# ArmingLou/seed-vc

Hardware: AMD Instinct MI355X
Metric: mel_frames_per_sec (higher is better)
Workload: dtype f16; 1 GPU; seed-uvit-tat-xlsr-tiny CFM 25 steps cfg 0.7 + HiFT, batch 64 x (P=430,S=430) per GPU; batch_per_gpu=64, global_batch=64, prompt_frames=430, diffusion_steps=25, vocoder_precision=fp16p8, lanes_per_gpu=2, parallelism=utterance-sharded x1, audio gather on rank 0

## Files before the change

### include/seedvc_hip.h

```cpp
#ifndef SEEDVC_HIP_H
#define SEEDVC_HIP_H

#include <stdint.h>

#ifdef __cplusplus
extern "C" {
#endif

#define SVC_ABI_VERSION 1

typedef struct svc_tensor_desc {
    const char* name;
    const float* data;
    int ndim;
    int64_t shape[4];
} svc_tensor_desc_t;

typedef struct svc_dit_config {
    int version;
    int hidden_dim, num_heads, depth, in_channels, content_dim, style_dim;
    int final_layer_type;
    int time_as_token, style_as_token, uvit_skip_connection, long_skip_connection, style_condition;
    int wn_hidden_dim, wn_num_layers, wn_kernel_size, wn_dilation_rate;
} svc_dit_config_t;
// ... 65 lines not shown
    int in_channels, base_channels, nb_harmonics, sampling_rate;
    float nsf_alpha, nsf_sigma, nsf_voiced_threshold;
    int num_upsamples, upsample_rates[4], upsample_kernel_sizes[4];
    int istft_n_fft, istft_hop;
    int num_kernels, resblock_kernel_sizes[4], resblock_dilation_sizes[4][3];
    int source_resblock_kernel_sizes[4], source_resblock_dilation_sizes[4][3];
    float lrelu_slope, audio_limit;
    int f0_cond_channels;
    int precision;
} svc_hift_config_t;
typedef struct svc_hift svc_hift_t;
int svc_hift_create(const svc_hift_config_t* cfg, const svc_tensor_desc_t* weights, int n_weights,
                    void* stream, svc_hift_t** out);
void svc_hift_destroy(svc_hift_t* m);
int svc_hift_forward(svc_hift_t* m, const float* mel, const float* f0, const float* phase0, const float* noise,
                     int B, int S, float* out, float* f0_out, void* stream);
int svc_hift_forward_ragged(svc_hift_t* m, const float* mel, const int32_t* lens, const float* f0, const float* phase0,
                            const float* noise, int B, int S, float* out, float* f0_out, void* stream);
int svc_hift_forward_seeded(svc_hift_t* m, const float* mel, const int32_t* lens, const float* f0, const uint64_t* seeds, int B,
                            int S, float* out, float* f0_out, void* stream);
int svc_hift_noise_draws(uint64_t seed, int NH, long n, float* phase0, float* noise, void* stream);
int svc_bigvgan_set_microbatch(svc_bigvgan_t* m, int utterances);
int svc_hift_set_microbatch(svc_hift_t* m, int utterances);

typedef struct svc_ar_config {
    int dim, n_head, n_local_heads, head_dim, n_layer, intermediate_size, vocab_size, max_seq_len;
    float rope_base, norm_eps;
} svc_ar_config_t;
typedef struct svc_ar svc_ar_t;
int svc_ar_create(const svc_ar_config_t* cfg, const svc_tensor_desc_t* weights, int n_weights, void* stream, svc_ar_t** out);
void svc_ar_destroy(svc_ar_t* m);
int svc_ar_reset(svc_ar_t* m, void* stream);
int svc_ar_forward_generate(svc_ar_t* m, const float* x, int S, const int64_t* input_pos, const int64_t* kv_pos,
                            float* logits_out, void* stream);
int svc_ar_decode_step(svc_ar_t* m, const float* x, int set_pos, int64_t input_pos, int64_t kv_pos, float* logits_out,
                       void* stream);
int svc_ar_generate(svc_ar_t* m, const float* x_prefill, int S, const int64_t* input_pos, const int64_t* kv_pos,
                    const float* exp_noise, int max_new, int min_tokens_before_eos, float temperature, float top_p,
                    float repetition_penalty, int check_every, int32_t* tokens_out, int32_t* n_tokens, void* stream);
int svc_ar_set_max_batch(svc_ar_t* m, int max_batch, void* stream);
int svc_ar_prefill_slot(svc_ar_t* m, int slot, const float* x, int S, const int64_t* input_pos, const int64_t* kv_pos,
                        float* logits_out, void* stream);
int svc_ar_decode_step_batch(svc_ar_t* m, int B, const float* x, int set_pos, const int64_t* input_pos, const int64_t* kv_pos,
                             float* logits_out, void* stream);
int svc_ar_generate_batch(svc_ar_t* m, int B, const float* x_prefill, const int32_t* S, const int64_t* input_pos,
                          const int64_t* kv_pos, const float* exp_noise, int max_new, int min_tokens_before_eos, float temperature,
// ... 428 lines not shown
```

### seed-vc_amd/_lib.py

```python
import ctypes as C
import os

import torch

_HERE = os.path.dirname(os.path.abspath(__file__))
LIB_PATH = os.path.join(_HERE, "libseedvc_hip.so")

EXPORTS = [
    "svc_abi_version", "svc_last_error",
    "svc_dit_create", "svc_dit_destroy", "svc_dit_set_microbatch", "svc_dit_set_fused_min_rows", "svc_dit_set_fused_seams", "svc_dit_fused_available", "svc_dit_set_graphs", "svc_cfm_sample", "svc_dit_forward",
    "svc_cfm_sample_seeded", "svc_cfm_noise_draws", "svc_cfm_sample_rows", "svc_cfm_rows_plan", "svc_hift_forward_seeded", "svc_hift_noise_draws",
    "svc_bigvgan_create", "svc_bigvgan_destroy", "svc_bigvgan_forward", "svc_bigvgan_forward_ragged", "svc_bigvgan_set_microbatch",
    "svc_hift_create", "svc_hift_destroy", "svc_hift_forward", "svc_hift_forward_ragged", "svc_hift_set_microbatch",
    "svc_anti_alias_act_fwd",
    "svc_ar_create", "svc_ar_destroy", "svc_ar_reset", "svc_ar_forward_generate", "svc_ar_decode_step", "svc_ar_sample", "svc_ar_generate",
    "svc_ar_set_max_batch", "svc_ar_prefill_slot", "svc_ar_decode_step_batch", "svc_ar_generate_batch",
    "svc_ar_generate_batch_seeded", "svc_ar_exp_draws", "svc_v2_assemble_cond", "svc_mel_strip_prompt",
    "svc_ar_prefill_batch", "svc_ar_set_prefill_rows", "svc_ar_prefill_passes", "svc_ar_admit", "svc_ar_run", "svc_ar_retire",
    "svc_ar_session_active",
    "svc_lr_create", "svc_lr_destroy", "svc_lr_forward", "svc_crossfade",
    "svc_chunks_gather_cond", "svc_chunks_assemble", "svc_sola_step", "svc_rt_push", "svc_rt_push_tiles", "svc_rt_ring_floats",
    "svc_rt_out", "svc_rt_push_gated", "svc_rt_out_dev", "svc_rt_pitch_state_words", "svc_rt_pitch",
    "svc_rt_pitch_cache_words", "svc_rt_pitch_ring_words", "svc_rt_pitch_win",
    "svc_vad_create", "svc_vad_destroy", "svc_vad_rows", "svc_vad_history", "svc_vad_state_floats", "svc_vad_scores", "svc_vad_detect",
    "svc_vad_step",
    "svc_campplus_create", "svc_campplus_destroy", "svc_campplus_forward", "svc_kaldi_fbank_frames", "svc_kaldi_fbank",
    "svc_kaldi_fbank_ragged", "svc_campplus_forward_ragged",
    "svc_mel_create", "svc_mel_destroy", "svc_mel_frames", "svc_mel_forward", "svc_mel_forward_ragged", "svc_mel_min_len",
    "svc_resampler_create", "svc_resampler_destroy", "svc_resample_len", "svc_resampler_tile", "svc_resample",
    "svc_rmvpe_create", "svc_rmvpe_destroy", "svc_rmvpe_frames", "svc_rmvpe_min_len", "svc_rmvpe_set_plane_budget", "svc_rmvpe_set_timing", "svc_rmvpe_last_timing", "svc_rmvpe_mel",
    "svc_rmvpe_salience", "svc_rmvpe_decode", "svc_rmvpe_f0", "svc_f0_adjust",
    "svc_whisper_create", "svc_whisper_destroy", "svc_whisper_n_windows", "svc_whisper_rows", "svc_whisper_set_window_group",
    "svc_whisper_set_timing", "svc_whisper_last_timing", "svc_whisper_mel", "svc_whisper_encode", "svc_whisper_content",
    "svc_w2v_create", "svc_w2v_destroy", "svc_w2v_frames", "svc_w2v_n_windows", "svc_w2v_rows", "svc_w2v_set_window_group",
    "svc_w2v_set_timing", "svc_w2v_last_timing", "svc_w2v_normalize", "svc_w2v_features", "svc_w2v_posconv", "svc_w2v_encode",
    "svc_w2v_content", "svc_w2v_create_ex",
# ... 389 lines not shown
```

### seed-vc_amd/csrc/attention.hip

```cpp
#include <stdlib.h>

#include <type_traits>

#include "common.h"

namespace svc {
namespace {

constexpr int KT = 64;
constexpr int ROWB = 128;

__device__ __forceinline__ int lds_off(int row, int c16) { return row * ROWB + ((c16 ^ ((row >> 1) & 7)) << 4); }

__device__ __forceinline__ half_t out16(float acc, float inv) {
    float r = acc * inv;
    asm volatile("" : "+v"(r));
    return (half_t)r;
}

template <int QT, bool VPERM, bool OUT32 = false>
__global__ __launch_bounds__(256) void attn_kernel(const AttnParams p) {
    constexpr int BQ = 64 * QT;
    constexpr int NS = 3;
    __shared__ __attribute__((aligned(16))) char smem[NS * 2 * KT * ROWB];
    const int tid = threadIdx.x, lane = tid & 63, wave = tid >> 6;
    const int fr = lane & 15, fq = lane >> 4;
    const int nblk = gridDim.x, bid = blockIdx.x;
    const int xq = nblk >> 3, xr = nblk & 7, xcd = bid & 7;
    const int lid = (xcd < xr ? xcd * (xq + 1) : xr * (xq + 1) + (xcd - xr) * xq) + (bid >> 3);
    const int nqt = (p.Tq - p.q_start + BQ - 1) / BQ;
    const int qt_idx = lid % nqt;
    const int sh_idx = lid / nqt;
    const int h = sh_idx % p.H, seq = sh_idx / p.H;
    const int q0 = p.q_start + qt_idx * BQ + wave * 16 * QT;
    const long row_base = (long)seq * p.seq_rows;
    const int kv_len = p.kv_len ? p.kv_len[seq] : p.kv_len_const;
    const int n_kt = (kv_len + KT - 1) / KT;

    half8 qf[QT][2];
#pragma unroll
    for (int qt = 0; qt < QT; ++qt) {
        int qr = q0 + qt * 16 + fr;
        qr = qr < p.seq_rows ? qr : p.seq_rows - 1;
        const half_t* src = p.q + (row_base + qr) * p.ld_qk + h * 64 + fq * 8;
// ... 23 lines not shown
    const half_t* kcol[2];
    const half_t* vp[2];
#pragma unroll
    for (int j = 0; j < 2; ++j) {
        srow[j] = (wave * 2 + j) * 8 + (lane >> 3);
        const int cs = (lane & 7) ^ ((srow[j] >> 1) & 7);
        kcol[j] = p.k + row_base * p.ld_qk + h * 64 + cs * 8;
        vp[j] = p.vt + (long)seq * p.vt_seq_stride + (long)(h * 64 + srow[j]) * p.vt_ld + cs * 8;
    }
    auto issue_tile = [&](int kt) {
        char* kb = smem + (kt % NS) * 2 * KT * ROWB + wave_u * 2048;
#pragma unroll
        for (int j = 0; j < 2; ++j) {
            int kr = kt * KT + srow[j];
            kr = kr < p.seq_rows ? kr : p.seq_rows - 1;
            __builtin_amdgcn_global_load_lds((gptr_t)(kcol[j] + (long)kr * p.ld_qk), (lptr_t)(kb + j * 1024), 16, 0, 0);
            __builtin_amdgcn_global_load_lds((gptr_t)(vp[j] + kt * KT), (lptr_t)(kb + KT * ROWB + j * 1024), 16, 0, 0);
        }
    };
#pragma unroll
    for (int s_ = 0; s_ < NS - 1; ++s_)
        if (s_ < n_kt) issue_tile(s_);

    auto tile = [&](const int kt, auto mask_tag) {
        constexpr bool MASK = decltype(mask_tag)::value;
        wait_tiles<NS - 2, 4>(n_kt - 1 - kt);
        asm volatile("s_barrier" ::: "memory");
        if (kt + NS - 1 < n_kt) issue_tile(kt + NS - 1);
        const char* kb = smem + (kt % NS) * 2 * KT * ROWB;
        const char* vb = kb + KT * ROWB;

        float4v acc_s[4][QT];
#pragma unroll
        for (int i = 0; i < 4; ++i)
#pragma unroll
            for (int j = 0; j < QT; ++j) acc_s[i][j] = (float4v){-m_run[j], -m_run[j], -m_run[j], -m_run[j]};
#pragma unroll
        for (int ks = 0; ks < 2; ++ks) {
#pragma unroll
            for (int mt = 0; mt < 4; ++mt) {
                const half8 kf = *reinterpret_cast<const half8*>(kb + lds_off(mt * 16 + fr, ks * 4 + fq));
#pragma unroll
                for (int qt = 0; qt < QT; ++qt)
                    acc_s[mt][qt] = __builtin_amdgcn_mfma_f32_16x16x32_f16(kf, qf[qt][ks], acc_s[mt][qt], 0, 0, 0);
            }
        }
        if constexpr (MASK) {
#pragma unroll
            for (int mt = 0; mt < 4; ++mt)
#pragma unroll
                for (int r = 0; r < 4; ++r) {
                    const int key = kt * KT + mt * 16 + fq * 4 + r;
                    if (key >= kv_len) {
#pragma unroll
                        for (int qt = 0; qt < QT; ++qt) acc_s[mt][qt][r] = -1e30f;
                    }
                }
        }
#pragma unroll
        for (int qt = 0; qt < QT; ++qt) {
            float a = -1e30f;
#pragma unroll
            for (int mt = 0; mt < 4; ++mt)
                a = fmaxf(a, fmaxf(fmaxf(acc_s[mt][qt][0], acc_s[mt][qt][1]), fmaxf(acc_s[mt][qt][2], acc_s[mt][qt][3])));
            if (__builtin_expect(kt == 0 || __any(a > THR), 0)) {
                a = fmaxf(a, __shfl_xor(a, 16));
                a = fmaxf(a, __shfl_xor(a, 32));
                const float delta = kt == 0 ? a : (a > THR ? a : 0.f);
                const float alpha = __builtin_amdgcn_exp2f(-delta);
                m_run[qt] += delta;
                acc_l[qt] *= alpha;
#pragma unroll
                for (int dt = 0; dt < 4; ++dt) acc_o[dt][qt] *= alpha;
#pragma unroll
                for (int mt = 0; mt < 4; ++mt) acc_s[mt][qt] -= delta;
            }
        }
#pragma unroll
        for (int ks = 0; ks < 2; ++ks) {
            half8 pf[QT];
#pragma unroll
            for (int qt = 0; qt < QT; ++qt) {
                u32x4 u;
#pragma unroll
                for (int hh = 0; hh < 2; ++hh) {
                    const float4v sv = acc_s[2 * ks + hh][qt];
                    const float e0 = __builtin_amdgcn_exp2f(sv[0]), e1 = __builtin_amdgcn_exp2f(sv[1]);
                    const float e2 = __builtin_amdgcn_exp2f(sv[2]), e3 = __builtin_amdgcn_exp2f(sv[3]);
                    u[2 * hh] = __builtin_bit_cast(unsigned, __builtin_amdgcn_cvt_pkrtz(e0, e1));
                    u[2 * hh + 1] = __builtin_bit_cast(unsigned, __builtin_amdgcn_cvt_pkrtz(e2, e3));
                }
                pf[qt] = __builtin_bit_cast(half8, u);
                acc_l[qt] = __builtin_amdgcn_mfma_f32_16x16x32_f16(ones_f, pf[qt], acc_l[qt], 0, 0, 0);
            }
#pragma unroll
            for (int dt = 0; dt < 4; ++dt) {
                const int d = dt * 16 + fr;
                half8 vf;
                if constexpr (VPERM) {
                    vf = *reinterpret_cast<const half8*>(vb + lds_off(d, ks * 4 + fq));
                } else {
                    const int base = lds_off(d, ks * 4 + (fq >> 1)) + (fq & 1) * 8;
                    const int base2 = lds_off(d, ks * 4 + 2 + (fq >> 1)) + (fq & 1) * 8;
                    const half4 v0 = *reinterpret_cast<const half4*>(vb + base);
                    const half4 v1 = *reinterpret_cast<const half4*>(vb + base2);
#pragma unroll
                    for (int e = 0; e < 4; ++e) { vf[e] = v0[e]; vf[4 + e] = v1[e]; }
                }
#pragma unroll
                for (int qt = 0; qt < QT; ++qt)
                    acc_o[dt][qt] = __builtin_amdgcn_mfma_f32_16x16x32_f16(vf, pf[qt], acc_o[dt][qt], 0, 0, 0);
            }
        }
    };
    const bool ragged = (kv_len % KT) != 0;
    const int n_full = ragged ? n_kt - 1 : n_kt;
    for (int kt = 0; kt < n_full; ++kt) tile(kt, std::false_type{});
    if (ragged) tile(n_kt - 1, std::true_type{});
    asm volatile("s_waitcnt vmcnt(0)" ::: "memory");

#pragma unroll
    for (int qt = 0; qt < QT; ++qt) {
        const float l = __shfl(acc_l[qt][0], fr);
        const float inv = l > 0.f ? 1.0f / l : 0.f;
        const int qr = q0 + qt * 16 + fr;
        if constexpr (OUT32) {
          if (qr < p.Tq) {
            float* dst = p.out32 + (row_base + qr) * p.ld_out + h * 64 + fq * 4;
#pragma unroll
            for (int dt = 0; dt < 4; ++dt)
                *reinterpret_cast<float4v*>(dst + dt * 16) =
                    (float4v){acc_o[dt][qt][0] * inv, acc_o[dt][qt][1] * inv, acc_o[dt][qt][2] * inv, acc_o[dt][qt][3] * inv};
          }
        } else if (qr < p.Tq) {
            half_t* dst = p.out + (row_base + qr) * p.ld_out + h * 64 + fq * 4;
#pragma unroll
            for (int dt = 0; dt < 4; ++dt) {
                half4 o = {out16(acc_o[dt][qt][0], inv), out16(acc_o[dt][qt][1], inv),
                           out16(acc_o[dt][qt][2], inv), out16(acc_o[dt][qt][3], inv)};
                *reinterpret_cast<half4*>(dst + dt * 16) = o;
            }
// ... 223 lines not shown
int attention_permute_vt(half_t* vt, long rows, long vt_ld, int mode, hipStream_t st) {
    SVC_REQUIRE(vt_ld % 32 == 0, "attention_permute_vt: vt_ld must be a multiple of 32");
    const long n = rows * (vt_ld / 32);
    hipLaunchKernelGGL(vt_permute_kernel, dim3(cdiv(n, 256)), dim3(256), 0, st, vt, rows, vt_ld, mode);
    SVC_CHECK_HIP(hipGetLastError());
    return 0;
}

int attention_launch(const AttnParams& p, hipStream_t st) {
    SVC_REQUIRE(p.n_seq > 0 && p.H > 0 && p.Tq > 0 && p.q_start >= 0 && p.q_start < p.Tq, "attention shape");
    SVC_REQUIRE(p.vt_ld % 64 == 0 && p.ld_qk % 8 == 0 && p.ld_out % 4 == 0, "attention alignment");
    SVC_REQUIRE(p.Tq <= p.seq_rows, "attention: Tq <= seq_rows");
    SVC_REQUIRE(p.vt_perm >= 0 && p.vt_perm <= 2 && p.qt_form >= 0 && p.qt_form <= 2, "attention: vt_perm and qt_form are 0 .. 2");
    SVC_REQUIRE((p.out != nullptr) != (p.out32 != nullptr), "attention: exactly one of out and out32");
    SVC_REQUIRE(p.kv_len || (p.kv_len_const >= 0 && p.kv_len_const <= p.seq_rows && round_up(p.kv_len_const, 64) <= p.vt_ld),
                "attention: kv_len_const within seq_rows, and within vt_ld when rounded up to a key tile");
    const int g128 = cdiv(p.Tq - p.q_start, 128) * p.H * p.n_seq;
    const bool prof = prof_enabled();
    if (prof) prof_begin(PROF_ATTN, st);
    static const int qt_env = [] { const char* e = getenv("SVC_ATTN_QT"); return e ? atoi(e) : 0; }();
    const dim3 g64(cdiv(p.Tq - p.q_start, 64) * p.H * p.n_seq);
    const bool small = p.qt_form ? p.qt_form == 1 : (qt_env == 1 || (qt_env == 0 && g128 <= 256));
    const bool small32 = p.qt_form ? p.qt_form == 1 : g128 <= 256;
    if (p.out32) {
        if (p.vt_perm == 2) {
            if (small32) hipLaunchKernelGGL((attn32_kernel<2, 3, true, true, true>), g64, dim3(128), 0, st, p);
            else hipLaunchKernelGGL((attn32_kernel<4, 3, true, true, true>), dim3(g128), dim3(256), 0, st, p);
        } else if (small) {
            if (p.vt_perm) hipLaunchKernelGGL((attn_kernel<1, true, true>), g64, dim3(256), 0, st, p);
            else hipLaunchKernelGGL((attn_kernel<1, false, true>), g64, dim3(256), 0, st, p);
        } else {
            if (p.vt_perm) hipLaunchKernelGGL((attn_kernel<2, true, true>), dim3(g128), dim3(256), 0, st, p);
            else hipLaunchKernelGGL((attn_kernel<2, false, true>), dim3(g128), dim3(256), 0, st, p);
        }
    } else if (p.vt_perm == 2) {
        if (small32) hipLaunchKernelGGL((attn32_kernel<2>), g64, dim3(128), 0, st, p);
        else hipLaunchKernelGGL((attn32_kernel<4>), dim3(g128), dim3(256), 0, st, p);
    } else if (small) {
        if (p.vt_perm) hipLaunchKernelGGL((attn_kernel<1, true>), g64, dim3(256), 0, st, p);
        else hipLaunchKernelGGL((attn_kernel<1, false>), g64, dim3(256), 0, st, p);
    } else {
        if (p.vt_perm) hipLaunchKernelGGL((attn_kernel<2, true>), dim3(g128), dim3(256), 0, st, p);
        else hipLaunchKernelGGL((attn_kernel<2, false>), dim3(g128), dim3(256), 0, st, p);
    }
    SVC_CHECK_HIP(hipGetLastError());
    if (prof) {
        const double tk = p.kv_len ? p.seq_rows : p.kv_len_const;
        prof_end(PROF_ATTN, 4.0 * p.n_seq * p.H * (double)(p.Tq - p.q_start) * tk * 64.0,
                 2.0 * p.n_seq * p.H * 64.0 * (2.0 * (p.Tq - p.q_start) + 2.0 * tk), st);
    }
    return 0;
}

}
```

### seed-vc_amd/csrc/common.h

```cpp
#pragma once
#include <atomic>
#include <hip/hip_runtime.h>
#include <stdint.h>
#include <stdio.h>
#include <string>

namespace svc {

typedef _Float16 half_t;
typedef _Float16 half8 __attribute__((ext_vector_type(8)));
typedef _Float16 half4 __attribute__((ext_vector_type(4)));
typedef _Float16 half2v __attribute__((ext_vector_type(2)));
typedef float float4v __attribute__((ext_vector_type(4)));
typedef unsigned int u32x4 __attribute__((ext_vector_type(4)));

void set_error(const std::string& msg);
const char* get_error();

#define SVC_CHECK_HIP(expr)                                                                  \
    do {                                                                                     \
        hipError_t _e = (expr);                                                              \
        if (_e != hipSuccess) {                                                              \
            svc::set_error(std::string(#expr) + ": " + hipGetErrorString(_e) + " at " + __FILE__ + \
                           ":" + std::to_string(__LINE__));                                  \
// ... 104 lines not shown
#undef SVC_ACT8
}

struct KGemmParams {
    const void* a_ptr[KG_MAX_TAPS];
    long a_ld[KG_MAX_TAPS];
    int a_shift[KG_MAX_TAPS];
    int a_ktiles[KG_MAX_TAPS];
    int n_taps;
    int Lout, a_seq_rows, a_off, a_stride, a_len, pad_mode;
    int reflect_min;
    const int* seq_len;
    const int* a_seq_map;
    const void* zero_page;
    float prof_flop_scale;
    int debug;
    int group_n;
    const void* w;
    long ldw;
    int M, N;
    int c_seq_rows, c_off;
    float* c32; long ldc32;
    half_t* c16; long ldc16;
    const float* post_a; const float* post_ib; int post_n; half_t* c16_lo;
    const float* bias;
    const float* rowvec; long ld_rowvec;
    const float* gate;   long ld_gate;
    const float* res;    long ldres;
    const float* res2;   long ldres2;
    float out_scale;
    int act; float act_slope;
    int post_relu;
    int vec_ok;
    const float* rope;
    int rope_D;
    float q_scale;
    half_t* vt; long vt_seq_stride; long vt_ld;
    int vt_mode;
};

int kgemm_launch(const KGemmParams& p, int dtype , int epi, hipStream_t st);
int kgemm_big_launch(const KGemmParams& p, int epi, hipStream_t st);

struct KConvParams {
    const void* a_hi; const void* a_lo;
    const void* w; long ldw;
// ... 100 lines not shown
```

### seed-vc_amd/csrc/conv_util.h

```cpp
#pragma once
#include <stdlib.h>
#include <string.h>

#include <string>

#include "model_util.h"

namespace svc {

struct ConvW {
    void* w = nullptr;
    float* bias = nullptr;
    long ldw = 0;
    int k = 0, cin_pad = 0, cout = 0, cout_pad = 0, dtype = 0, vd = 0;
    void* w8 = nullptr;
    long ldw8 = 0;
    int w8_exp = 0;
    int stride = 0;
};

inline int gdt(int vd) { return vd == 1 ? 1 : 0; }
inline bool is_split(int vd) { return vd == 2 || vd == 3; }
inline int cpad(int c, int vd) { return (int)round_up(c, ktile_elems(gdt(vd))); }
inline size_t vesize(int vd) { return esize(gdt(vd)); }
// ... 178 lines not shown
                          p.N >= kconv_min_n();
    SVC_REQUIRE((!r.p8 && !r.c16_lo_fmt) || (kconv_ok && (!r.p8 || conv_p8_ok(w, r.Lout, r.dilation))),
                "conv1d_run: the fp8-pair operand format needs the resident-tile kernel");
    if (kconv_ok) {
        KConvParams q;
        memset(&q, 0, sizeof(q));
        q.a_hi = r.a.hi; q.a_lo = r.a.lo; q.w = r.p8 ? w.w8 : w.w; q.ldw = r.p8 ? w.ldw8 : w.ldw; q.bias = w.bias;
        q.B = r.B; q.Lin = r.Lin; q.Lout = r.Lout; q.N = p.N; q.cin_pad = w.cin_pad; q.k = w.k; q.dil = r.dilation;
        q.pad_left = r.pad_left; q.nsub = r.p8 ? 2 : nsub; q.w8_exp = w.w8_exp; q.c16_lo_fmt = r.c16_lo_fmt;
        q.c_seq_rows = p.c_seq_rows; q.c_off = p.c_off;
        q.c32 = r.c32; q.ldc32 = r.ldc32; q.c16 = r.c16; q.c16_lo = r.c16_lo; q.ldc16 = r.ldc16;
        q.post_a = r.post_a; q.post_ib = r.post_ib; q.post_n = r.post_n;
        q.res = r.res; q.ldres = r.ldres; q.res2 = r.res2; q.ldres2 = r.ldres2;
        q.out_scale = r.out_scale; q.act = r.act; q.act_slope = r.act_slope;
        q.seq_len = r.seq_len;
        q.bm = r.bm; q.took = r.took;
        return kconv_launch(q, st);
    }
    if (r.took) *r.took = 0;
    return kgemm_launch(p, w.dtype, KG_EPI_STORE, st);
}

inline int convT_run(const ConvW& w, ActBuf a, int B, int L, float* c32, int c_rows_q, int c_off_q, hipStream_t st,
                     const int* seq_len = nullptr) {
    KGemmParams p;
    memset(&p, 0, sizeof(p));
    const int nsub = is_split(w.vd) ? 3 : 1;
    p.M = B * L;
    p.N = w.stride * w.cout_pad;
    p.Lout = L;
    p.a_seq_rows = L;
    p.a_len = L;
    p.seq_len = seq_len;
    p.a_stride = 1;
    p.pad_mode = KG_PAD_ZERO;
    p.n_taps = 3 * nsub;
    const int kt = w.cin_pad / ktile_elems(w.dtype);
    for (int t = 0; t < 3; ++t)
        for (int sub = 0; sub < nsub; ++sub) {
            const int i = t * nsub + sub;
            p.a_ptr[i] = sub == 2 ? a.lo : a.hi;
            p.a_ld[i] = w.cin_pad;
            p.a_ktiles[i] = kt;
            p.a_shift[i] = t - 1;
        }
    p.w = w.w;
    p.ldw = w.ldw;
    p.bias = w.bias;
    p.c_seq_rows = c_rows_q ? c_rows_q : L;
    p.c_off = c_off_q;
    p.c32 = c32;
    p.ldc32 = p.N;
    p.vec_ok = 1;
    p.prof_flop_scale = 1.0f / nsub;
    return kgemm_launch(p, w.dtype, KG_EPI_STORE, st);
}

}
```

### seed-vc_amd/csrc/kgemm.hip

```cpp
#include "kgemm_tile.h"

namespace svc {

namespace {

template <typename T, int EPI>
int launch_wide(const KGemmParams& p, hipStream_t st) {
    const int v = p.debug & 0xF0;
    if (v == 0x10) return launch_one<T, 128, 128, 64, 3, EPI>(p, st);
    if (v == 0x20) return launch_one<T, 128, 128, 64, 4, EPI>(p, st);
    if (v == 0x80) return launch_one<T, 256, 128, 128, 3, EPI>(p, st);
    if (v == 0x40) return launch_one<T, 128, 128, 128, 2, EPI>(p, st);
    if (v == 0x50) return launch_one<T, 64, 64, 128, 2, EPI, 4>(p, st);
    if (v == 0x60) return launch_one<T, 64, 64, 128, 4, EPI, 4>(p, st);
    if (v == 0x70) return launch_one<T, 64, 128, 128, 2, EPI, 4>(p, st);
    if (v == 0xB0) return launch_one<T, 256, 128, 64, 3, EPI, 4>(p, st);
    if constexpr (sizeof(T) == 2) {
        const bool big_ok = p.N % 256 == 0 && (EPI != KG_EPI_QKV_ROPE || (2 * p.rope_D) % 256 == 0);
        if (v == 0x90 && big_ok) return kgemm_big_launch(p, EPI, st);
    }
    long kt = 0;
    for (int t = 0; t < p.n_taps; ++t) kt += p.a_ktiles[t];
    const long gm64 = cdiv(p.M, 64);
    if (gm64 * cdiv(p.N, 64) <= 768) {
// ... 4 lines not shown
    if (kt <= 8) return launch_one<T, 128, 128, 64, 3, EPI>(p, st);
    static const int tall = [] { const char* e = getenv("SVC_KGEMM_TALL"); return e ? atoi(e) : 3; }();
    if (sizeof(T) == 2 && kt >= 12 && p.N >= 768 && p.N % 128 == 0 && (long)cdiv(p.M, 256) * (p.N / 128) >= 512 &&
        ((EPI == KG_EPI_SWIGLU && (tall & 1) && p.N >= 2048) || (EPI == KG_EPI_QKV_ROPE && (tall & 2)) || (EPI == KG_EPI_STORE && (tall & 4))))
        return launch_one<T, 256, 128, 64, 3, EPI, 4>(p, st);
    return launch_one<T, 128, 128, 128, 2, EPI>(p, st);
}

template <typename T, int EPI>
int launch_bn(const KGemmParams& p, hipStream_t st) {
    if (p.N <= 32) return launch_one<T, 128, 32, 128, 2, EPI>(p, st);
    if (p.N <= 64) return launch_one<T, 128, 64, 128, 2, EPI>(p, st);
    return launch_wide<T, EPI>(p, st);
}

}

int kgemm_dispatch(const KGemmParams& p, int dtype, int epi, hipStream_t st);

int kgemm_launch(const KGemmParams& p_in, int dtype, int epi, hipStream_t st) {
    const KGemmParams& p0 = p_in;
    SVC_REQUIRE(p0.n_taps >= 1 && p0.n_taps <= KG_MAX_TAPS, "tap count");
    SVC_REQUIRE(p0.Lout > 0 && p0.M >= 0 && p0.N > 0, "shape");
    if (p0.M == 0) return 0;
    DeviceState* ds = device_state();
    if (!ds) return 1;
    KGemmParams p = p_in;
    p.zero_page = ds->zero_page;
    static const int env_variant = [] { const char* e = getenv("SVC_KGEMM_VARIANT"); return e ? atoi(e) & 0xF0 : 0; }();
    if (!(p.debug & 0xF0)) p.debug |= env_variant;
    static const int env_group = [] { const char* e = getenv("SVC_KGEMM_GROUP"); return e ? atoi(e) : 8; }();
    p.group_n = env_group;
    const bool prof = prof_enabled();
    const int cls = dtype == 0 ? PROF_KGEMM_F16 : PROF_KGEMM_F32;
    if (prof) prof_begin(cls, st);
    const int rc = kgemm_dispatch(p, dtype, epi == KG_EPI_STORE && p.act == KG_ACT_GELU ? KG_EPI_STORE_GELU : epi, st);
    if (prof) {
        long kt = 0;
        for (int t = 0; t < p.n_taps; ++t) kt += p.a_ktiles[t];
        const double K = (double)kt * (dtype == 0 ? 64 : 32);
        const double es = dtype == 0 ? 2 : 4;
        double bytes = ((double)p.M * K / (p.n_taps > 1 && p.a_ptr[0] == p.a_ptr[p.n_taps - 1] ? p.n_taps : 1) + (double)p.N * K) * es;
        bytes += (double)p.M * p.N * ((p.c32 ? 4 : 0) + (p.c16 ? 2 : 0) + (p.res ? 4 : 0) + (p.res2 ? 4 : 0));
        const unsigned long long tag = ((unsigned long long)p.M << 40) | ((unsigned long long)(p.N & 0xFFFFF) << 20) |
                                       ((unsigned long long)((long)K & 0xFFFF) << 4) | (unsigned)(epi & 0xF);
        prof_end(cls, 2.0 * p.M * (double)p.N * K * (p.prof_flop_scale > 0.f ? p.prof_flop_scale : 1.0), bytes, st, tag);
// ... 26 lines not shown
```

### seed-vc_amd/csrc/kgemm_tile.h

```cpp
#pragma once
#include <stdlib.h>

#include "common.h"

namespace svc {

namespace {

template <int BM, int BN, int RB, int NS, int NWV>
struct Geo {
    static constexpr int NW = NWV;
    static constexpr int NT = NW * 64;
    static constexpr int WAVES_N = (BN >= 128) ? 2 : 1;
    static constexpr int WAVES_M = NW / WAVES_N;
    static constexpr int WTM = BM / WAVES_M;
    static constexpr int WTN = BN / WAVES_N;
    static constexpr int TM = WTM / 16;
    static constexpr int TN = WTN / 16;
    static constexpr int EPI_LD = WTN + 4;
    static constexpr int NSTAGE = NS;
    static constexpr int STAGE_BYTES = (BM + BN) * RB;
    static constexpr int LDS_AB = NSTAGE * STAGE_BYTES;
    static constexpr int EPI_FULL = NW * WTM * EPI_LD * 4;
    static constexpr int EP = (EPI_FULL <= LDS_AB || TM == 1) ? 1 : ((EPI_FULL / 2 <= LDS_AB || TM == 2) ? 2 : 4);
// ... 334 lines not shown
                }
            }
            return;
        }
    }

    if constexpr (!DIRECT) {
        __syncthreads();
    constexpr int CW = 8;
    constexpr int CPR = G::WTN / CW;
    constexpr int TMP = G::TM / G::EP;
    constexpr int ROWS_P = TMP * 16;
    constexpr int NCH = ROWS_P * CPR / 64;
    static_assert(ROWS_P * CPR % 64 == 0, "epilogue chunking");
    float* ep = reinterpret_cast<float*>(smem) + wave * ROWS_P * G::EPI_LD;
    static_assert(64 % CPR == 0, "a lane keeps its columns");
    const int cc = lane % CPR, row0 = lane / CPR;
    const int n = n0 + wn0 + cc * CW;
    const int nv = (p.N - n) < CW ? (p.N - n) : CW;
    const int n_ld = nv > 0 ? n : 0;
    const bool rv_vec = p.vec_ok && (p.N & 7) == 0 && (p.ld_rowvec & 3) == 0 && (reinterpret_cast<uintptr_t>(p.rowvec) & 15) == 0;
    const bool gt_vec = p.vec_ok && (p.N & 7) == 0 && (p.ld_gate & 3) == 0 && (reinterpret_cast<uintptr_t>(p.gate) & 15) == 0;
    const bool sn_vec = n + CW <= p.post_n && ((reinterpret_cast<uintptr_t>(p.post_a) | reinterpret_cast<uintptr_t>(p.post_ib)) & 15) == 0;
    float cb[CW];
#pragma unroll
    for (int j = 0; j < CW; ++j) cb[j] = 0.f;

#pragma unroll
    for (int pass = 0; pass < G::EP; ++pass) {
        const int prow0 = pass * ROWS_P;
        long orow_[NCH];
        int seq_[NCH], pos_[NCH];
        bool ok_[NCH];
        float4v rs0[NCH], rs1[NCH];
#pragma unroll
        for (int i = 0; i < NCH; ++i) {
            const int m = m0 + wm0 + prow0 + row0 + (64 / CPR) * i;
            ok_[i] = (m < p.M) & (nv > 0);
            const int mm = ok_[i] ? m : 0;
            seq_[i] = mm / p.Lout;
            pos_[i] = mm - seq_[i] * p.Lout;
            orow_[i] = (long)seq_[i] * p.c_seq_rows + p.c_off + pos_[i];
        }
        if (p.res && p.vec_ok) {
#pragma unroll
            for (int i = 0; i < NCH; ++i) {
// ... 76 lines not shown
                        for (int j = 0; j < 8; ++j) if (j < nv) v[j] *= gv[j];
                    }
                }
                if (p.vec_ok) {
                    if (p.res) {
#pragma unroll
                        for (int j = 0; j < 4; ++j) { v[j] += rs0[i][j]; v[4 + j] += rs1[i][j]; }
                    }
                    if (p.out_scale != 0.f) {
#pragma unroll
                        for (int j = 0; j < 8; ++j) v[j] *= p.out_scale;
                    }
                    if (p.res2) {
                        const float4v q0 = *reinterpret_cast<const float4v*>(p.res2 + orow * p.ldres2 + n);
                        const float4v q1 = *reinterpret_cast<const float4v*>(p.res2 + orow * p.ldres2 + n + 4);
#pragma unroll
                        for (int j = 0; j < 4; ++j) { v[j] += q0[j]; v[4 + j] += q1[j]; }
                    }
                    if (p.post_relu) {
#pragma unroll
                        for (int j = 0; j < 8; ++j) v[j] = fmaxf(v[j], 0.f);
                    }
                    if (p.c32) {
                        *reinterpret_cast<float4v*>(p.c32 + orow * p.ldc32 + n) = (float4v){v[0], v[1], v[2], v[3]};
                        *reinterpret_cast<float4v*>(p.c32 + orow * p.ldc32 + n + 4) = (float4v){v[4], v[5], v[6], v[7]};
                    }
                    if (p.post_a) {
                        float lo[8], ca[8], cib[8];
                        if (sn_vec) {
#pragma unroll
                            for (int q4 = 0; q4 < 2; ++q4) {
                                const float4v a4 = *reinterpret_cast<const float4v*>(p.post_a + n + q4 * 4);
                                const float4v i4 = *reinterpret_cast<const float4v*>(p.post_ib + n + q4 * 4);
#pragma unroll
                                for (int j = 0; j < 4; ++j) { ca[q4 * 4 + j] = a4[j]; cib[q4 * 4 + j] = i4[j]; }
                            }
                        } else {
#pragma unroll
                            for (int j = 0; j < 8; ++j) {
                                const int nn = n + j < p.post_n ? n + j : (p.post_n > 0 ? p.post_n - 1 : 0);
                                ca[j] = p.post_n > 0 ? p.post_a[nn] : 0.f;
                                cib[j] = p.post_n > 0 ? p.post_ib[nn] : 0.f;
                            }
                        }
#pragma unroll
                        for (int j = 0; j < 8; ++j) {
                            const float t = v[j] + cib[j] * sin_sq(ca[j] * v[j]);
                            const float sv = n + j < p.post_n ? t : 0.f;
                            const half_t h = (half_t)sv;
                            v[j] = sv;
                            lo[j] = sv - (float)h;
                        }
                        if (p.c16_lo) *reinterpret_cast<uint4*>(p.c16_lo + orow * p.ldc16 + n) = pack8(lo);
                    }
                    if (p.c16) *reinterpret_cast<uint4*>(p.c16 + orow * p.ldc16 + n) = pack8(v);
                } else {
                    for (int j = 0; j < nv; ++j) {
                        float o = v[j];
                        if (p.res) o += p.res[orow * p.ldres + n + j];
                        if (p.out_scale != 0.f) o *= p.out_scale;
                        if (p.res2) o += p.res2[orow * p.ldres2 + n + j];
                        if (p.post_relu) o = fmaxf(o, 0.f);
                        if (p.c32) p.c32[orow * p.ldc32 + n + j] = o;
                        if (p.post_a) {
                            const int nn = n + j;
                            o = nn < p.post_n ? o + p.post_ib[nn] * sin_sq(p.post_a[nn] * o) : 0.f;
                            if (p.c16_lo) p.c16_lo[orow * p.ldc16 + n + j] = (half_t)(o - (float)(half_t)o);
                        }
                        if (p.c16) p.c16[orow * p.ldc16 + n + j] = (half_t)o;
                    }
                }
            }
        }
    }
        return;
    }

    const int n = n0 + wn0 + CW * fq;
    if (n >= p.N) return;
    const int nv = (p.N - n) < CW ? (p.N - n) : CW;
    const bool full = nv == CW && p.vec_ok;
    long orow_[G::TM];
    int seq_[G::TM], pos_[G::TM];
    bool ok_[G::TM];
#pragma unroll
    for (int mt = 0; mt < G::TM; ++mt) {
// ... 110 lines not shown
```

### seed-vc_amd/csrc/vocoder.hip

```cpp
#include <math.h>
#include <stdlib.h>
#include <string.h>

#include <algorithm>
#include <functional>
#include <vector>

#include "conv_util.h"
#include "noise.h"

using namespace svc;

namespace {


__global__ void snake_params_kernel(const float* alpha, const float* beta, float* a, float* inv_b, int C, int mode) {
    const int c = blockIdx.x * blockDim.x + threadIdx.x;
    if (c >= C) return;
    float al = alpha[c], be = beta ? beta[c] : alpha[c];
    if (mode != 2) { al = expf(al); be = expf(be); }
    a[c] = al;
    inv_b[c] = 1.0f / (be + 1e-9f);
}

// ... 569 lines not shown
    for (int d = 0; d < ndil; ++d) {
        rb->dil[d] = dils[d];
        const std::string ds = std::to_string(d);
        if (pack_conv1d(sd, p + ".convs1." + ds, ch, ch, k, true, dtype, ar, st, &rb->c1[d])) return 1;
        if (pack_conv1d(sd, p + ".convs2." + ds, ch, ch, k, true, dtype, ar, st, &rb->c2[d])) return 1;
        if (bigvgan_names) {
            const std::string a1 = p + ".activations." + std::to_string(2 * d) + ".act";
            const std::string a2 = p + ".activations." + std::to_string(2 * d + 1) + ".act";
            if (make_snake(sd, a1 + ".alpha", has_beta ? a1 + ".beta" : "", ch, snake_mode, ar, st, &rb->a1[d])) return 1;
            if (make_snake(sd, a2 + ".alpha", has_beta ? a2 + ".beta" : "", ch, snake_mode, ar, st, &rb->a2[d])) return 1;
        } else {
            if (make_snake(sd, p + ".activations1." + ds + ".alpha", "", ch, 2, ar, st, &rb->a1[d])) return 1;
            if (make_snake(sd, p + ".activations2." + ds + ".alpha", "", ch, 2, ar, st, &rb->a2[d])) return 1;
        }
    }
    return 0;
}
}

struct svc_hift {
    svc_hift_config_t cfg;
    int dtype;
    int microbatch = 0;
    Arena wts, ws;
    ConvW f0_convs[5];
    float *f0_lin_w, *f0_lin_b, *src_lin_w, *src_lin_b;
    ConvW conv_pre, conv_post, ups[2], src_down[2];
    ResBlockW src_rb[2];
    std::vector<ResBlockW> blocks;
    int up_total;
    int cap_B = 0, cap_S = 0;
    ActOut mel_a, act_a, act_b, stft_a;
    void *f0_a, *f0_b;
    float *f0_buf, *s_buf, *stft32, *x, *y, *t, *xsum, *si, *post, *frames;
    double* prefix;
    RaggedPlan plan;
    int device = -1;
    Arena seed_ar;
    unsigned long long* d_seeds = nullptr;
    float* d_phase0 = nullptr;
    int seed_cap = 0;

    int reserve(int B, int S, hipStream_t st);
    int run(const float* mel, const float* f0, const float* phase0, const float* noise, int B, int S, float* out, float* f0_out,
            hipStream_t st, const RaggedMB* rg = nullptr, const unsigned long long* seeds = nullptr);
    int forward(const float* mel, const float* f0, const float* phase0, const float* noise, const unsigned long long* seeds, int B,
// ... 115 lines not shown
        if (ew_cl(stft32, stft_a, vd, (long)B * F, ld18, ld18, 3, 0.f, st)) return 1;
        stft_in = stft_a.in();
    }
    if (mel_to_cl(mel, mel_a, vd, rm, B, cfg.in_channels, S, cpad(cfg.in_channels, dtype), st)) return 1;
    {
        ConvRun r;
        r.a = mel_a.in(); r.B = B; r.Lin = S; r.Lout = S; r.pad_left = 3;
        r.c32 = xsum; r.ldc32 = cpad(bc, dtype);
        r.seq_len = len0; r.seq_kconv = true;
        if (conv1d_run(conv_pre, r, st)) return 1;
    }
    int ch = bc;
    long L = S;
    const int nk = cfg.num_kernels;
    for (int i = 0; i < cfg.num_upsamples; ++i) {
        const bool last_up = i == cfg.num_upsamples - 1;
        if (ew_cl(xsum, act_a, vd, (long)B * L, ch, cpad(ch, dtype), 2, cfg.lrelu_slope, st)) return 1;
        const int u = cfg.upsample_rates[i];
        const long Lnew = L * u + (last_up ? 1 : 0);
        ch /= 2;
        const int ld = cpad(ch, dtype);
        if (last_up) {
            const size_t a_step = (size_t)L * ups[i].cin_pad * vesize(dtype);
            for (int b = 0; b < B; ++b) {
                ActBuf ab;
                ab.hi = (const char*)act_a.hi + b * a_step;
                ab.lo = (const char*)act_a.lo + b * a_step;
                const int Lb = rg ? (int)((long)rg->h_len0[b] * (L / S)) : (int)L;
                if (Lb == 0) continue;
                if (convT_run(ups[i], ab, 1, Lb, x + ((long)b * Lnew + 1) * ld, 0, 0, st)) return 1;
            }
            hipLaunchKernelGGL(copy_row_kernel, dim3(cdiv((long)B * ld, 256)), dim3(256), 0, st, x, B, (int)Lnew, ld, 2, 0);
            SVC_CHECK_HIP(hipGetLastError());
        } else {
            if (convT_run(ups[i], act_a.in(), B, (int)L, x, 0, 0, st, rg ? rg->len[i] : nullptr)) return 1;
        }
        L = Lnew;
        const int* len_i = rg ? rg->len[i + 1] : nullptr;
        {
            ConvRun r;
            r.a = stft_in; r.B = B; r.Lin = F; r.Lout = (int)L;
            const int dk = src_down[i].k;
            if (dk == 1) { r.stride = 1; r.pad_left = 0; }
            else { r.stride = dk / 2; r.pad_left = dk / 4; }
            r.c32 = si; r.ldc32 = ld;
            r.seq_len = len_f;
// ... 154 lines not shown
        if (pack_conv1d(sd, "source_downs." + std::to_string(i), ch, cfg->istft_n_fft + 2, dk, true, m->dtype, m->wts, st,
                        &m->src_down[i])) return fail();
        if (pack_resblock(sd, "source_resblocks." + std::to_string(i), ch, cfg->source_resblock_kernel_sizes[i],
                          cfg->source_resblock_dilation_sizes[i], 3, m->dtype, 2, false, false, m->wts, st, &m->src_rb[i]))
            return fail();
        for (int j = 0; j < cfg->num_kernels; ++j) {
            ResBlockW rb;
            if (pack_resblock(sd, "resblocks." + std::to_string(i * cfg->num_kernels + j), ch, cfg->resblock_kernel_sizes[j],
                              cfg->resblock_dilation_sizes[j], 3, m->dtype, 2, false, false, m->wts, st, &rb)) return fail();
            m->blocks.push_back(rb);
        }
    }
    if (pack_conv1d(sd, "conv_post", cfg->istft_n_fft + 2, ch, 7, true, m->dtype, m->wts, st, &m->conv_post)) return fail();
    if (hipStreamSynchronize(st) != hipSuccess) { set_error("sync failed"); return fail(); }
    *out = m;
    return 0;
}

void svc_hift_destroy(svc_hift_t* m) { delete m; }

int svc_hift_set_microbatch(svc_hift_t* m, int utterances) {
    SVC_REQUIRE(m && utterances >= 0, "bad argument");
    m->microbatch = utterances;
    return 0;
}

int svc_hift_forward(svc_hift_t* m, const float* mel, const float* f0, const float* phase0, const float* noise, int B, int S,
                     float* out, float* f0_out, void* stream) {
    SVC_REQUIRE(m && mel && phase0 && noise && out && B >= 1 && S >= 1, "bad argument");
    return m->forward(mel, f0, phase0, noise, nullptr, B, S, out, f0_out, (hipStream_t)stream);
}

int svc_hift_forward_ragged(svc_hift_t* m, const float* mel, const int32_t* lens, const float* f0, const float* phase0,
                            const float* noise, int B, int S, float* out, float* f0_out, void* stream) {
    SVC_REQUIRE(m && mel && lens && phase0 && noise && out && B >= 1 && S >= 1, "bad argument");
    return m->forward_ragged(mel, lens, f0, phase0, noise, nullptr, B, S, out, f0_out, (hipStream_t)stream);
}

int svc_hift_forward_seeded(svc_hift_t* m, const float* mel, const int32_t* lens, const float* f0, const uint64_t* seeds, int B,
                            int S, float* out, float* f0_out, void* stream) {
    SVC_REQUIRE(m && mel && out, "null argument");
    SVC_REQUIRE(seeds, "svc_hift_forward_seeded: seeds is NULL (HOST [B], one per utterance)");
    SVC_REQUIRE(B >= 1 && S >= 1, "svc_hift_forward_seeded: B and S must be at least 1");
    SVC_REQUIRE((long)S * m->up_total <= 0x7fffffffL, "svc_hift_forward_seeded: the sample index is a 32-bit counter word");
    SVC_REQUIRE(current_device() == m->device, "this handle was created on another device (make it current before the call)");
    if (lens)
// ... 296 lines not shown
```

### seed-vc_amd/vocoder.py

```python
import ctypes as C
import math

import torch

from . import _lib
from .specs import bigvgan_total_upsample, hift_total_upsample


PRECISIONS = {"fp32": 0, "fp16": 1, "fp16x3": 2, "fp16p8": 3}


class BigVGAN:
    def __init__(self, h, state_dict, device="cuda:0", precision="fp16p8"):
        self.h = h
        self.device = torch.device(device)
        self.total_up = bigvgan_total_upsample(h)
        c = _lib.BigVGANConfig()
        c.num_mels = h["num_mels"]
        c.upsample_initial_channel = h["upsample_initial_channel"]
        c.num_upsamples = len(h["upsample_rates"])
        c.num_kernels = len(h["resblock_kernel_sizes"])
        for i, (u, k) in enumerate(zip(h["upsample_rates"], h["upsample_kernel_sizes"])):
            c.upsample_rates[i], c.upsample_kernel_sizes[i] = u, k
        for j, (k, d) in enumerate(zip(h["resblock_kernel_sizes"], h["resblock_dilation_sizes"])):
# ... 62 lines not shown
        c.istft_n_fft, c.istft_hop = cfg["istft_n_fft"], cfg["istft_hop"]
        c.num_kernels = len(cfg["resblock_kernel_sizes"])
        for j, (k, d) in enumerate(zip(cfg["resblock_kernel_sizes"], cfg["resblock_dilation_sizes"])):
            c.resblock_kernel_sizes[j] = k
            for e in range(3):
                c.resblock_dilation_sizes[j][e] = d[e]
        for j, (k, d) in enumerate(zip(cfg["source_resblock_kernel_sizes"], cfg["source_resblock_dilation_sizes"])):
            c.source_resblock_kernel_sizes[j] = k
            for e in range(3):
                c.source_resblock_dilation_sizes[j][e] = d[e]
        c.lrelu_slope, c.audio_limit = cfg["lrelu_slope"], cfg["audio_limit"]
        c.f0_cond_channels = cfg["f0_cond_channels"]
        c.precision = PRECISIONS[precision]
        self._h = C.c_void_p()
        with torch.cuda.device(self.device):
            descs, n, keep = _lib.make_descs(state_dict, self.device)
            _lib.check(_lib.lib().svc_hift_create(C.byref(c), descs, n, _lib.stream_ptr(), C.byref(self._h)))
            torch.cuda.current_stream().synchronize()
        del keep

    def set_microbatch(self, n):
        _lib.check(_lib.lib().svc_hift_set_microbatch(self._h, int(n)))

    @torch.inference_mode()
    def __call__(self, x, f0=None, phase0=None, noise=None, return_f0=False, lens=None, seeds=None):
        B, _, S = x.shape
        if seeds is not None and (phase0 is not None or noise is not None):
            raise ValueError("HiFT: give seeds or phase0 / noise, not both")
        seeds_keep = _lib.seeds_host(seeds, B, "HiFT") if seeds is not None else None
        if lens is not None:
            lens = _lib.int_list(lens)
            if len(lens) != B:
                raise ValueError(f"HiFT: lens has {len(lens)} entries, the batch has {B} utterances")
        nh = self.cfg["nb_harmonics"] + 1
        Lw = S * self.total_up
        dev = self.device
        with torch.cuda.device(dev):
            mel = _lib.f32c(x, dev)
            if seeds is None:
                if phase0 is None:
                    phase0 = (torch.rand(B, nh, 1, device=dev) * 2 - 1) * math.pi
                if noise is None:
                    noise = torch.randn(B, nh, Lw, device=dev)
                phase0, noise = _lib.f32c(phase0, dev), _lib.f32c(noise, dev)
            f0t = _lib.f32c(f0, dev) if f0 is not None else None
            out = torch.empty(B, Lw, device=dev, dtype=torch.float32)
# ... 37 lines not shown
```

Before: 141,600 mel-frames/s.

## Halve masked attention tail tile work and batch the HiFT last upsample

Adds a reduced-work mode for the ragged final key tile in the attention kernel. When 32 or fewer keys remain, it computes only two of the four 16-key score subtiles and one PV k-step. This mode is on by default and can be turned off with an environment variable. Separately, the last HiFT transposed-conv upsample now runs as one batched GEMM with a per-sequence output stride, instead of a per-utterance loop of launches. The risks are correctness around the tail mask and the new strided store path, which is restricted to plain fp32 stores.

```diff
diff --git a/include/seedvc_hip.h b/include/seedvc_hip.h
--- a/include/seedvc_hip.h
+++ b/include/seedvc_hip.h
@@ -111,6 +111,7 @@
 int svc_hift_noise_draws(uint64_t seed, int NH, long n, float* phase0, float* noise, void* stream);
 int svc_bigvgan_set_microbatch(svc_bigvgan_t* m, int utterances);
 int svc_hift_set_microbatch(svc_hift_t* m, int utterances);
+int svc_hift_set_upsample_batched(svc_hift_t* m, int on);
 
 typedef struct svc_ar_config {
     int dim, n_head, n_local_heads, head_dim, n_layer, intermediate_size, vocab_size, max_seq_len;
diff --git a/seed-vc_amd/_lib.py b/seed-vc_amd/_lib.py
--- a/seed-vc_amd/_lib.py
+++ b/seed-vc_amd/_lib.py
@@ -12,6 +12,7 @@
     "svc_cfm_sample_seeded", "svc_cfm_noise_draws", "svc_cfm_sample_rows", "svc_cfm_rows_plan", "svc_hift_forward_seeded", "svc_hift_noise_draws",
     "svc_bigvgan_create", "svc_bigvgan_destroy", "svc_bigvgan_forward", "svc_bigvgan_forward_ragged", "svc_bigvgan_set_microbatch",
     "svc_hift_create", "svc_hift_destroy", "svc_hift_forward", "svc_hift_forward_ragged", "svc_hift_set_microbatch",
+    "svc_hift_set_upsample_batched",
     "svc_anti_alias_act_fwd",
     "svc_ar_create", "svc_ar_destroy", "svc_ar_reset", "svc_ar_forward_generate", "svc_ar_decode_step", "svc_ar_sample", "svc_ar_generate",
     "svc_ar_set_max_batch", "svc_ar_prefill_slot", "svc_ar_decode_step_batch", "svc_ar_generate_batch",
diff --git a/seed-vc_amd/csrc/attention.hip b/seed-vc_amd/csrc/attention.hip
--- a/seed-vc_amd/csrc/attention.hip
+++ b/seed-vc_amd/csrc/attention.hip
@@ -19,7 +19,7 @@
 }
 
 template <int QT, bool VPERM, bool OUT32 = false>
-__global__ __launch_bounds__(256) void attn_kernel(const AttnParams p) {
+__global__ __launch_bounds__(256) void attn_kernel(const AttnParams p, const int tail32) {
     constexpr int BQ = 64 * QT;
     constexpr int NS = 3;
     __shared__ __attribute__((aligned(16))) char smem[NS * 2 * KT * ROWB];
@@ -89,23 +89,26 @@
     for (int s_ = 0; s_ < NS - 1; ++s_)
         if (s_ < n_kt) issue_tile(s_);
 
-    auto tile = [&](const int kt, auto mask_tag) {
-        constexpr bool MASK = decltype(mask_tag)::value;
+    auto tile = [&](const int kt, auto mode_tag) {
+        constexpr int MODE = decltype(mode_tag)::value;
+        constexpr bool MASK = MODE != 0;
+        constexpr int NMT = MODE == 2 ? 2 : 4;
+        constexpr int NKS = MODE == 2 ? 1 : 2;
         wait_tiles<NS - 2, 4>(n_kt - 1 - kt);
         asm volatile("s_barrier" ::: "memory");
         if (kt + NS - 1 < n_kt) issue_tile(kt + NS - 1);
         const char* kb = smem + (kt % NS) * 2 * KT * ROWB;
         const char* vb = kb + KT * ROWB;
 
-        float4v acc_s[4][QT];
-#pragma unroll
-        for (int i = 0; i < 4; ++i)
+        float4v acc_s[NMT][QT];
+#pragma unroll
+        for (int i = 0; i < NMT; ++i)
 #pragma unroll
             for (int j = 0; j < QT; ++j) acc_s[i][j] = (float4v){-m_run[j], -m_run[j], -m_run[j], -m_run[j]};
 #pragma unroll
         for (int ks = 0; ks < 2; ++ks) {
 #pragma unroll
-            for (int mt = 0; mt < 4; ++mt) {
+            for (int mt = 0; mt < NMT; ++mt) {
                 const half8 kf = *reinterpret_cast<const half8*>(kb + lds_off(mt * 16 + fr, ks * 4 + fq));
 #pragma unroll
                 for (int qt = 0; qt < QT; ++qt)
@@ -114,7 +117,7 @@
         }
         if constexpr (MASK) {
 #pragma unroll
-            for (int mt = 0; mt < 4; ++mt)
+            for (int mt = 0; mt < NMT; ++mt)
 #pragma unroll
                 for (int r = 0; r < 4; ++r) {
                     const int key = kt * KT + mt * 16 + fq * 4 + r;
@@ -128,7 +131,7 @@
         for (int qt = 0; qt < QT; ++qt) {
             float a = -1e30f;
 #pragma unroll
-            for (int mt = 0; mt < 4; ++mt)
+            for (int mt = 0; mt < NMT; ++mt)
                 a = fmaxf(a, fmaxf(fmaxf(acc_s[mt][qt][0], acc_s[mt][qt][1]), fmaxf(acc_s[mt][qt][2], acc_s[mt][qt][3])));
             if (__builtin_expect(kt == 0 || __any(a > THR), 0)) {
                 a = fmaxf(a, __shfl_xor(a, 16));
@@ -140,11 +143,11 @@
 #pragma unroll
                 for (int dt = 0; dt < 4; ++dt) acc_o[dt][qt] *= alpha;
 #pragma unroll
-                for (int mt = 0; mt < 4; ++mt) acc_s[mt][qt] -= delta;
-            }
-        }
-#pragma unroll
-        for (int ks = 0; ks < 2; ++ks) {
+                for (int mt = 0; mt < NMT; ++mt) acc_s[mt][qt] -= delta;
+            }
+        }
+#pragma unroll
+        for (int ks = 0; ks < NKS; ++ks) {
             half8 pf[QT];
 #pragma unroll
             for (int qt = 0; qt < QT; ++qt) {
@@ -182,8 +185,11 @@
     };
     const bool ragged = (kv_len % KT) != 0;
     const int n_full = ragged ? n_kt - 1 : n_kt;
-    for (int kt = 0; kt < n_full; ++kt) tile(kt, std::false_type{});
-    if (ragged) tile(n_kt - 1, std::true_type{});
+    for (int kt = 0; kt < n_full; ++kt) tile(kt, std::integral_constant<int, 0>{});
+    if (ragged) {
+        if (tail32 && kv_len - (n_kt - 1) * KT <= 32) tile(n_kt - 1, std::integral_constant<int, 2>{});
+        else tile(n_kt - 1, std::integral_constant<int, 1>{});
+    }
     asm volatile("s_waitcnt vmcnt(0)" ::: "memory");
 
 #pragma unroll
@@ -453,26 +459,28 @@
     const dim3 g64(cdiv(p.Tq - p.q_start, 64) * p.H * p.n_seq);
     const bool small = p.qt_form ? p.qt_form == 1 : (qt_env == 1 || (qt_env == 0 && g128 <= 256));
     const bool small32 = p.qt_form ? p.qt_form == 1 : g128 <= 256;
+    const char* t32 = getenv("SVC_ATTN_TAIL32");
+    const int tail32 = !(t32 && t32[0] == '0');
     if (p.out32) {
         if (p.vt_perm == 2) {
             if (small32) hipLaunchKernelGGL((attn32_kernel<2, 3, true, true, true>), g64, dim3(128), 0, st, p);
             else hipLaunchKernelGGL((attn32_kernel<4, 3, true, true, true>), dim3(g128), dim3(256), 0, st, p);
         } else if (small) {
-            if (p.vt_perm) hipLaunchKernelGGL((attn_kernel<1, true, true>), g64, dim3(256), 0, st, p);
-            else hipLaunchKernelGGL((attn_kernel<1, false, true>), g64, dim3(256), 0, st, p);
+            if (p.vt_perm) hipLaunchKernelGGL((attn_kernel<1, true, true>), g64, dim3(256), 0, st, p, tail32);
+            else hipLaunchKernelGGL((attn_kernel<1, false, true>), g64, dim3(256), 0, st, p, tail32);
         } else {
-            if (p.vt_perm) hipLaunchKernelGGL((attn_kernel<2, true, true>), dim3(g128), dim3(256), 0, st, p);
-            else hipLaunchKernelGGL((attn_kernel<2, false, true>), dim3(g128), dim3(256), 0, st, p);
+            if (p.vt_perm) hipLaunchKernelGGL((attn_kernel<2, true, true>), dim3(g128), dim3(256), 0, st, p, tail32);
+            else hipLaunchKernelGGL((attn_kernel<2, false, true>), dim3(g128), dim3(256), 0, st, p, tail32);
         }
     } else if (p.vt_perm == 2) {
         if (small32) hipLaunchKernelGGL((attn32_kernel<2>), g64, dim3(128), 0, st, p);
         else hipLaunchKernelGGL((attn32_kernel<4>), dim3(g128), dim3(256), 0, st, p);
     } else if (small) {
-        if (p.vt_perm) hipLaunchKernelGGL((attn_kernel<1, true>), g64, dim3(256), 0, st, p);
-        else hipLaunchKernelGGL((attn_kernel<1, false>), g64, dim3(256), 0, st, p);
+        if (p.vt_perm) hipLaunchKernelGGL((attn_kernel<1, true>), g64, dim3(256), 0, st, p, tail32);
+        else hipLaunchKernelGGL((attn_kernel<1, false>), g64, dim3(256), 0, st, p, tail32);
     } else {
-        if (p.vt_perm) hipLaunchKernelGGL((attn_kernel<2, true>), dim3(g128), dim3(256), 0, st, p);
-        else hipLaunchKernelGGL((attn_kernel<2, false>), dim3(g128), dim3(256), 0, st, p);
+        if (p.vt_perm) hipLaunchKernelGGL((attn_kernel<2, true>), dim3(g128), dim3(256), 0, st, p, tail32);
+        else hipLaunchKernelGGL((attn_kernel<2, false>), dim3(g128), dim3(256), 0, st, p, tail32);
     }
     SVC_CHECK_HIP(hipGetLastError());
     if (prof) {
diff --git a/seed-vc_amd/csrc/common.h b/seed-vc_amd/csrc/common.h
--- a/seed-vc_amd/csrc/common.h
+++ b/seed-vc_amd/csrc/common.h
@@ -150,6 +150,7 @@
     int c_seq_rows, c_off;
     float* c32; long ldc32;
     half_t* c16; long ldc16;
+    long c_seq_stride;
     const float* post_a; const float* post_ib; int post_n; half_t* c16_lo;
     const float* bias;
     const float* rowvec; long ld_rowvec;
diff --git a/seed-vc_amd/csrc/conv_util.h b/seed-vc_amd/csrc/conv_util.h
--- a/seed-vc_amd/csrc/conv_util.h
+++ b/seed-vc_amd/csrc/conv_util.h
@@ -224,7 +224,7 @@
 }
 
 inline int convT_run(const ConvW& w, ActBuf a, int B, int L, float* c32, int c_rows_q, int c_off_q, hipStream_t st,
-                     const int* seq_len = nullptr) {
+                     const int* seq_len = nullptr, long c_seq_stride = 0) {
     KGemmParams p;
     memset(&p, 0, sizeof(p));
     const int nsub = is_split(w.vd) ? 3 : 1;
@@ -251,6 +251,7 @@
     p.bias = w.bias;
     p.c_seq_rows = c_rows_q ? c_rows_q : L;
     p.c_off = c_off_q;
+    p.c_seq_stride = c_seq_stride;
     p.c32 = c32;
     p.ldc32 = p.N;
     p.vec_ok = 1;
diff --git a/seed-vc_amd/csrc/kgemm.hip b/seed-vc_amd/csrc/kgemm.hip
--- a/seed-vc_amd/csrc/kgemm.hip
+++ b/seed-vc_amd/csrc/kgemm.hip
@@ -50,6 +50,9 @@
     const KGemmParams& p0 = p_in;
     SVC_REQUIRE(p0.n_taps >= 1 && p0.n_taps <= KG_MAX_TAPS, "tap count");
     SVC_REQUIRE(p0.Lout > 0 && p0.M >= 0 && p0.N > 0, "shape");
+    SVC_REQUIRE(p0.c_seq_stride == 0 || (epi == KG_EPI_STORE && p0.c32 && !p0.c16 && !p0.c16_lo && !p0.res && !p0.res2 &&
+                                         p0.c_seq_stride % 4 == 0 && p0.c_seq_stride >= (long)(p0.c_off + p0.Lout) * p0.ldc32),
+                "c_seq_stride: plain fp32 STORE only, a multiple of 4 floats that holds a sequence's rows");
     if (p0.M == 0) return 0;
     DeviceState* ds = device_state();
     if (!ds) return 1;
diff --git a/seed-vc_amd/csrc/kgemm_tile.h b/seed-vc_amd/csrc/kgemm_tile.h
--- a/seed-vc_amd/csrc/kgemm_tile.h
+++ b/seed-vc_amd/csrc/kgemm_tile.h
@@ -380,6 +380,7 @@
     const bool rv_vec = p.vec_ok && (p.N & 7) == 0 && (p.ld_rowvec & 3) == 0 && (reinterpret_cast<uintptr_t>(p.rowvec) & 15) == 0;
     const bool gt_vec = p.vec_ok && (p.N & 7) == 0 && (p.ld_gate & 3) == 0 && (reinterpret_cast<uintptr_t>(p.gate) & 15) == 0;
     const bool sn_vec = n + CW <= p.post_n && ((reinterpret_cast<uintptr_t>(p.post_a) | reinterpret_cast<uintptr_t>(p.post_ib)) & 15) == 0;
+    const long c_skip = p.c_seq_stride ? p.c_seq_stride - (long)p.c_seq_rows * p.ldc32 : 0;
     float cb[CW];
 #pragma unroll
     for (int j = 0; j < CW; ++j) cb[j] = 0.f;
@@ -502,8 +503,9 @@
                         for (int j = 0; j < 8; ++j) v[j] = fmaxf(v[j], 0.f);
                     }
                     if (p.c32) {
-                        *reinterpret_cast<float4v*>(p.c32 + orow * p.ldc32 + n) = (float4v){v[0], v[1], v[2], v[3]};
-                        *reinterpret_cast<float4v*>(p.c32 + orow * p.ldc32 + n + 4) = (float4v){v[4], v[5], v[6], v[7]};
+                        float* cd = p.c32 + orow * p.ldc32 + seq * c_skip + n;
+                        *reinterpret_cast<float4v*>(cd) = (float4v){v[0], v[1], v[2], v[3]};
+                        *reinterpret_cast<float4v*>(cd + 4) = (float4v){v[4], v[5], v[6], v[7]};
                     }
                     if (p.post_a) {
                         float lo[8], ca[8], cib[8];
@@ -541,7 +543,7 @@
                         if (p.out_scale != 0.f) o *= p.out_scale;
                         if (p.res2) o += p.res2[orow * p.ldres2 + n + j];
                         if (p.post_relu) o = fmaxf(o, 0.f);
-                        if (p.c32) p.c32[orow * p.ldc32 + n + j] = o;
+                        if (p.c32) p.c32[orow * p.ldc32 + seq * c_skip + n + j] = o;
                         if (p.post_a) {
                             const int nn = n + j;
                             o = nn < p.post_n ? o + p.post_ib[nn] * sin_sq(p.post_a[nn] * o) : 0.f;
diff --git a/seed-vc_amd/csrc/vocoder.hip b/seed-vc_amd/csrc/vocoder.hip
--- a/seed-vc_amd/csrc/vocoder.hip
+++ b/seed-vc_amd/csrc/vocoder.hip
@@ -615,6 +615,7 @@
     svc_hift_config_t cfg;
     int dtype;
     int microbatch = 0;
+    int upsample_batched = 1;
     Arena wts, ws;
     ConvW f0_convs[5];
     float *f0_lin_w, *f0_lin_b, *src_lin_w, *src_lin_b;
@@ -776,6 +777,9 @@
         const int ld = cpad(ch, dtype);
         if (last_up) {
             const size_t a_step = (size_t)L * ups[i].cin_pad * vesize(dtype);
+            if (upsample_batched) {
+                if (convT_run(ups[i], act_a.in(), B, (int)L, x + ld, 0, 0, st, rg ? rg->len[i] : nullptr, Lnew * ld)) return 1;
+            } else
             for (int b = 0; b < B; ++b) {
                 ActBuf ab;
                 ab.hi = (const char*)act_a.hi + b * a_step;
@@ -976,6 +980,12 @@
 int svc_hift_set_microbatch(svc_hift_t* m, int utterances) {
     SVC_REQUIRE(m && utterances >= 0, "bad argument");
     m->microbatch = utterances;
+    return 0;
+}
+
+int svc_hift_set_upsample_batched(svc_hift_t* m, int on) {
+    SVC_REQUIRE(m && (on == 0 || on == 1), "bad argument");
+    m->upsample_batched = on;
     return 0;
 }
 
diff --git a/seed-vc_amd/vocoder.py b/seed-vc_amd/vocoder.py
--- a/seed-vc_amd/vocoder.py
+++ b/seed-vc_amd/vocoder.py
@@ -108,6 +108,9 @@
     def set_microbatch(self, n):
         _lib.check(_lib.lib().svc_hift_set_microbatch(self._h, int(n)))
 
+    def set_upsample_batched(self, on):
+        _lib.check(_lib.lib().svc_hift_set_upsample_batched(self._h, int(on)))
+
     @torch.inference_mode()
     def __call__(self, x, f0=None, phase0=None, noise=None, return_f0=False, lens=None, seeds=None):
         B, _, S = x.shape
```

New measurement: 142,600 mel-frames/s, median of 6. Within noise of the previous version (+0.7%).
